# leggedrobotics/delora

Measured on AMD Instinct MI355X. Metric: training scan-pairs/sec, KITTI 64x2048 range images, higher is better.
Workload: dtype f32; 1 GPU; KITTI-shaped 64x2048, batch=8 pairs/GPU, raw scans of ~141k points (ragged, raster order), steps rotate over 8 distinct HBM-resident batches, online normals, ResNet pose CNN (11.9M params, identity-pretrained state), Adam; BASELINE configs[1]; global_batch=8, parallelism=dp1, cnn=fp32, cnn_impl=hip trunk: fp32 MFMA, fused Winograd F(2x2,3x3) + direct implicit GEMM, channels_last=False, hip_graph=False, distinct_batches=8, priming_steps=8

## Files before the change

delora_amd/_lib.py:

```python
import ctypes
import os

_HERE = os.path.dirname(os.path.abspath(__file__))
LIB_PATH = os.path.join(_HERE, "csrc", "libdelora_hip.so")
ABI_VERSION = 10


class DeloraHipError(RuntimeError):
    pass


class SensorStruct(ctypes.Structure):
    _fields_ = [("H", ctypes.c_int32), ("W", ctypes.c_int32),
                ("hfov0", ctypes.c_double), ("hfov1", ctypes.c_double),
                ("vfov0", ctypes.c_double), ("vfov1", ctypes.c_double)]


_vp, _i32, _i64, _u32, _f32, _sz = (ctypes.c_void_p, ctypes.c_int32, ctypes.c_int64, ctypes.c_uint32,
                                    ctypes.c_float, ctypes.c_size_t)
_SP = ctypes.POINTER(SensorStruct)

SIGNATURES = {
    "dl_abi_version": (_i32, []),
    "dl_last_error": (ctypes.c_char_p, []),
# ... 70 lines not shown
    "dl_channel_scale_bwd_act_nhwc_t": (_i32, [_vp, _vp, _vp, _i32, _i32, _i32, _i32, _i32, _vp, _vp]),
    "dl_tower_wide_drop_f32": (_i32, [_vp, _vp, ctypes.c_double, _i32, _i32, _i32, _i32, _i32, _vp, _vp]),
    "dl_tower_wide_drop_bwd_f32": (_i32, [_vp, _vp, _vp, ctypes.c_double, _i32, _i32, _i32, _i32, _i32, _i32, _vp, _vp]),
    "dl_mean_hw_nhwc_h": (_i32, [_vp, _i32, _i32, _i32, _i32, _vp, _vp]),
    "dl_mean_hw_bwd_act_h": (_i32, [_vp, _vp, _i32, _i32, _i32, _i32, _i32, _vp, _vp]),
    "dl_conv2d_wgrad_h_workspace_bytes": (_sz, [_i32, _i32, _i32, _i32, _i32, _i32, _i32, _i32]),
    "dl_conv2d_wgrad_nhwc_h": (_i32, [_vp, _vp, _vp, _vp, _i32, _i32, _i32, _i32, _i32, _i32, _i32, _i32, _i32, _vp]),
    "dl_wgrad_batch_plan": (_i64, [_vp, _vp, _i32, _i32, _i32, _vp]),
    "dl_wino_wgrad3x3_batch_workspace_bytes": (_sz, [_vp, _i32]),
    "dl_wino_wgrad3x3_batch_nhwc_f32": (_i32, [_vp, _i32, _vp, _vp]),
    "dl_conv2d_wgrad_batch_workspace_bytes": (_sz, [_vp, _i32]),
    "dl_conv2d_wgrad_batch_nhwc_f32": (_i32, [_vp, _i32, _vp, _vp]),
    "dl_conv2d_wgrad_batch_h_workspace_bytes": (_sz, [_vp, _i32]),
    "dl_conv2d_wgrad_batch_nhwc_h": (_i32, [_vp, _i32, _vp, _i32, _vp]),
    "dl_conv_plan_describe": (_i32, [_i32, _i32, _i32, _i32, _i32, _i32, _i32, _i32, _i32, _i32, _i32, _i32, ctypes.c_char_p, _sz]),
    "dl_profile_begin": (_i32, [_i32, ctypes.c_char_p]),
    "dl_profile_end": (_i32, [_vp, _i32, ctypes.POINTER(ctypes.c_int32), ctypes.POINTER(ctypes.c_int32)]),
    "dl_profile_pause": (_i32, [_i32]),
}


class WinoLayer(ctypes.Structure):
    _fields_ = [("w", ctypes.c_void_p), ("u_fwd", ctypes.c_void_p), ("u_bwd", ctypes.c_void_p), ("K", ctypes.c_int32), ("C", ctypes.c_int32)]


WINO_BATCH = 16


class HeadsParams(ctypes.Structure):
    _fields_ = [(n, ctypes.c_void_p) for n in ("fc_w", "fc_b", "r1_w", "r1_b", "r3_w", "r3_b", "t1_w", "t1_b", "t3_w", "t3_b")]
# ... 38 lines not shown
    rows = (ProfileRow * capacity)()
    n, untimed = ctypes.c_int32(), ctypes.c_int32()
    check(load().dl_profile_end(ctypes.cast(rows, ctypes.c_void_p), capacity, ctypes.byref(n), ctypes.byref(untimed)), "dl_profile_end")
    out = [{"name": rows[i].name.decode(), "launches": rows[i].launches, "ms": rows[i].ms, "flop": rows[i].flop, "bytes": rows[i].bytes}
           for i in range(min(n.value, capacity))]
    return out, untimed.value

PLAN_CONV, PLAN_DGRAD_STRIDED, PLAN_WINO_CONV, PLAN_WGRAD, PLAN_WGRAD_BATCH, PLAN_WINO_WGRAD, PLAN_WINO_WGRAD_BATCH = range(7)


def conv_plan(op, dtype, N, H, W, C, K, ksize=3, sh=1, sw=1, mode=0, cu_count=0):
    buf = ctypes.create_string_buffer(4096)
    check(load().dl_conv_plan_describe(int(op), int(dtype), int(N), int(H), int(W), int(C), int(K), int(ksize), int(sh), int(sw),
                                       int(mode), int(cu_count), buf, len(buf)), "dl_conv_plan_describe")
    return buf.value.decode().split("\n")


_lib = None


def load():
    global _lib
    if _lib is not None:
        return _lib
    if not os.path.exists(LIB_PATH):
        raise DeloraHipError(
            f"{LIB_PATH} is missing: build it with `python -c 'import __graft_entry__ as g; g.build()'` "
            f"or `make -C delora_amd/csrc`. The geometry path has no fallback implementation.")
    import torch
    try:
# ... 17 lines not shown
```

delora_amd/csrc/abi.hip:

```cpp
#include <stdarg.h>
#include <stdint.h>
#include <stdio.h>
#include <stdlib.h>
#include <string.h>
#include <cxxabi.h>

#include <atomic>
#include <map>
#include <mutex>
#include <string>
#include <vector>

#include "common.h"

thread_local char g_dl_err[256] = {0};

int dl_fail(int code, const char* fmt, ...) {
  va_list ap;
  va_start(ap, fmt);
  vsnprintf(g_dl_err, sizeof(g_dl_err), fmt, ap);
  va_end(ap);
  return code;
}

// ... 133 lines not shown
  free(full);
  char tail[96];
  const int m = snprintf(tail, sizeof(tail), " grid=%ux%ux%u block=%u", grid.x, grid.y, grid.z, block.x);
  dl_plan_append(tail, (size_t)m);
}

void dl_plan_note(const char* fmt, ...) {
  char text[96] = " ";
  va_list ap;
  va_start(ap, fmt);
  const int m = vsnprintf(text + 1, sizeof(text) - 1, fmt, ap);
  va_end(ap);
  if (m > 0) dl_plan_append(text, (size_t)(m < (int)sizeof(text) - 2 ? m + 1 : sizeof(text) - 1));
}

extern "C" int dl_abi_version(void) { return DL_ABI_VERSION; }
extern "C" const char* dl_last_error(void) { return g_dl_err; }

namespace {
struct ProfAgg { int launches = 0; double flop = 0, bytes = 0; std::vector<int> ev; };
struct Profiler {
  std::mutex mu;
  std::atomic<bool> open{false};
  std::atomic<bool> paused{false};
  std::vector<hipEvent_t> ev;
  int used = 0, skipped = 0;
  std::string only;
  std::map<std::string, ProfAgg> rows;
};
Profiler g_prof;
// ... 68 lines not shown
```

delora_amd/csrc/common.h:

```cpp
#pragma once
#include <hip/hip_runtime.h>
#include <stdint.h>

#include "../../include/delora_hip.h"

#define DL_WAVE 64
#define DL_BLOCK 256

struct SensorK {
  int H, W, HW;
  float hf0f, hspanf, wm1f;
  float vf0f, vspanf, hm1f;
  double hf0, hres, vf0, vres;
  float tol_u, tol_v;
};

static inline SensorK make_sensor(const dl_sensor* s) {
  SensorK k;
  k.H = s->H; k.W = s->W; k.HW = s->H * s->W;
  k.hf0f = (float)s->hfov0; k.hspanf = (float)(s->hfov1 - s->hfov0); k.wm1f = (float)(s->W - 1);
  k.vf0f = (float)s->vfov0; k.vspanf = (float)(s->vfov1 - s->vfov0); k.hm1f = (float)(s->H - 1);
  k.hf0 = s->hfov0; k.hres = (s->hfov1 - s->hfov0) / (double)(s->W - 1);
  k.vf0 = s->vfov0; k.vres = (s->vfov1 - s->vfov0) / (double)(s->H - 1);
  k.tol_u = (float)(3e-6 * fabs((double)k.wm1f / (double)k.hspanf) + 2.4e-7 * (double)s->W);
// ... 39 lines not shown
  p = __builtin_fmaf(p, t, 0.020650655031204224f);
  p = __builtin_fmaf(p, t, -0.05374353006482124f);
  p = __builtin_fmaf(p, t, 0.13331492245197296f);
  p = __builtin_fmaf(p, t, -0.3333328366279602f);
  const float lo = __builtin_fmaf(ax * t, p, ax);
  const float e = __builtin_amdgcn_exp2f(ax * 2.885390081777927f);
  const float hi = __builtin_fmaf(__builtin_amdgcn_rcpf(e + 1.f), -2.f, 1.f);
  return __builtin_copysignf(ax < 0.625f ? lo : hi, x);
}

extern thread_local char g_dl_err[256];
int dl_fail(int code, const char* fmt, ...);
int dl_check_launch(const char* what);
void dl_plan_batch(const int* tiles, const int* chunks, int n, int machines, int partial_cost, int* nslabs);
int dl_fill_words(void* p, uint32_t value, size_t n_words, hipStream_t st);

#include <hip/hip_ext.h>
struct DlProfTag {
  const char* kernel;
  const char* pass;
  int N, H, W, C, K;
  int ks, sh, sw;
  double flop;
  double bytes;
};
bool dl_prof_is_open();
void dl_prof_events(const DlProfTag& tag, hipEvent_t* e0, hipEvent_t* e1);

struct DlPlanSink {
  char* buf;
// ... 26 lines not shown
```

delora_amd/csrc/conv.hip:

```cpp
#include <type_traits>

#include "common.h"
#include "conv_geom.h"

typedef float f32x16 __attribute__((ext_vector_type(16)));
typedef float f32x4 __attribute__((ext_vector_type(4)));

__device__ __forceinline__ __amdgpu_buffer_rsrc_t cv_rsrc(const float* base, unsigned bytes) {
  return __builtin_amdgcn_make_buffer_rsrc(const_cast<float*>(base), 0, (int)bytes, 0x00020000);
}
__device__ __forceinline__ f32x4 cv_ld16(__amdgpu_buffer_rsrc_t rs, unsigned voff, unsigned soff) {
  return __builtin_bit_cast(f32x4, __builtin_amdgcn_raw_buffer_load_b128(rs, (int)voff, (int)soff, 0));
}
#define CV_ZERO_OFF 0x80000000u

#define CV_THREADS 256
#define CV_EPI_ADD 1u
#define CV_EPI_ACT 2u
#define CV_EPI_DACT 4u
#define CV_EPI_ADD_GRID 8u
#define CV_ACT_NONE 0
#define CV_ACT_TANH 1
#define CV_ACT_RELU 2

// ... 15 lines not shown
  if (act == CV_ACT_TANH) return dl_tanh(v);
  if (act == CV_ACT_RELU) return v < 0.f ? 0.f : v;
  return v;
}
__device__ __forceinline__ float cv_dact(float y, int act) {
  if (act == CV_ACT_TANH) return 1.f - y * y;
  if (act == CV_ACT_RELU) return y <= 0.f ? 0.f : 1.f;
  return 1.f;
}

__device__ __forceinline__ int cv_xcd_swizzle(int id, int n) {
  const int q = n / 8, r = n % 8, xcd = id % 8, k = id / 8;
  return (xcd < r ? xcd * (q + 1) : r * (q + 1) + (xcd - r) * q) + k;
}

template <int BM, int BN, int CK, int TW, class G, bool BT, int WGN>
#ifndef CV_MINWAVES
#define CV_MINWAVES 2
#endif
__global__ __launch_bounds__(CV_THREADS, CV_MINWAVES) void k_conv_f32(ConvArgs a) {
  constexpr int TH = BM / TW;
  constexpr int SH = G::ISH, SW = G::ISW;
  constexpr int RH = (TH - 1) * SH + G::EH, RW = (TW - 1) * SW + G::EW;
  constexpr int S = CK + 4;
  constexpr int TAPS = G::NT;
  constexpr int C4 = CK / 4;
  constexpr int IN_FLOATS = RH * RW * S;
  constexpr int W_FLOATS = BT ? TAPS * CK * BN : TAPS * BN * S;
  constexpr int NI = RH * RW * C4;
  constexpr int NW = BT ? CK * TAPS * (BN / 4) : BN * TAPS * C4;
  constexpr int NI_IT = (NI + CV_THREADS - 1) / CV_THREADS, NW_IT = (NW + CV_THREADS - 1) / CV_THREADS;
  constexpr int WGM = 4 / WGN;
  constexpr int WM = BM / 32 / WGM, WN = BN / 32 / WGN;
  static_assert(BM % TW == 0 && BM % (32 * WGM) == 0 && BN % (32 * WGN) == 0 && CK % 8 == 0, "tile shape");
  static_assert(TAPS > 0, "a stride phase without taps has no launch");
  static_assert((S / 4) % 2 == 1, "pixel stride must be 4*odd floats");
  constexpr int EPW = WN * 32, ES = EPW + 4;
  constexpr int LDS_HOLD = (BM == 256 && TW == 128 && CK == 8 && BT) ? 160 * 1024 / 3 / 4 + 16 : 0;
  constexpr int LDS_USED = IN_FLOATS + W_FLOATS > 4 * 32 * ES ? IN_FLOATS + W_FLOATS : 4 * 32 * ES;
  constexpr int LDS_FLOATS = LDS_USED > LDS_HOLD ? LDS_USED : LDS_HOLD;
  __shared__ __attribute__((aligned(16))) float lds[LDS_FLOATS];
  float* in_lds = lds;
  float* w_lds = lds + IN_FLOATS;

  const int tid = threadIdx.x, lane = tid & 63, wave = tid >> 6;
  const int li = lane & 31, half = lane >> 5;
  const int wm = wave / WGN, wn = wave % WGN;
  const int KT = a.K / BN;
  const int tiles_w = (a.Wo + TW - 1) / TW, tiles_h = (a.Ho + TH - 1) / TH;
  const int ntiles = a.N * tiles_h * tiles_w * KT;
  const int t = cv_xcd_swizzle(blockIdx.x, ntiles);
  const int kt = t % KT;
  int pt = t / KT;
  const int tw_i = pt % tiles_w; pt /= tiles_w;
  const int th_i = pt % tiles_h;
  const int n = pt / tiles_h;
  const int ho0 = th_i * TH, wo0 = tw_i * TW, k0 = kt * BN;
  const int h_base = ho0 * SH + G::H0, w_base = wo0 * SW + G::W0;
  const float* xn = a.x + (size_t)n * a.H * a.W * a.C;

  const unsigned x_bytes = (unsigned)(a.H * a.W * a.C) * 4u, w_bytes = (unsigned)(a.K * a.C * G::WTAPS) * 4u;
  const __amdgpu_buffer_rsrc_t x_rs = cv_rsrc(xn, x_bytes), w_rs = cv_rsrc(a.w, w_bytes);
  const unsigned x_zero = CV_ZERO_OFF;
  unsigned in_g[NI_IT];
  int in_l[NI_IT];
#pragma unroll
  for (int it = 0; it < NI_IT; ++it) {
    const int q = min(tid + it * CV_THREADS, NI - 1);
    const int c4 = q % C4, pc = q / C4;
    const int col = pc % RW, row = pc / RW;
    const int h = h_base + row;
    int w = w_base + col;
    const bool col_in = w >= 0 && w < a.W;
    w = w < 0 ? w + a.W : w;
    w = w >= a.W ? w - a.W : w;
    in_l[it] = pc * S + c4 * 4;
    in_g[it] = (h >= 0 && h < a.H && (a.wrap ? w < a.W : col_in)) ? (unsigned)((h * a.W + w) * a.C + c4 * 4) * 4u : x_zero;
  }
  unsigned w_g[NW_IT];
  int w_l[NW_IT];
#pragma unroll
  for (int it = 0; it < NW_IT; ++it) {
    const int q = min(tid + it * CV_THREADS, NW - 1);
    if (!BT) {
      const int c4 = q % C4, t2 = q / C4;
      const int tap = t2 % TAPS, kk = t2 / TAPS;
      w_g[it] = (unsigned)(((k0 + kk) * G::WTAPS + G::wt(tap)) * a.C + c4 * 4) * 4u;
      w_l[it] = (tap * BN + kk) * S + c4 * 4;
    } else {
      const int co4 = q % (BN / 4), t2 = q / (BN / 4);
      const int tap = t2 % TAPS, kr = t2 / TAPS;
      w_g[it] = (unsigned)((kr * G::WTAPS + G::wt(tap)) * a.K + k0 + co4 * 4) * 4u;
      w_l[it] = (tap * CK + kr) * BN + co4 * 4;
    }
  }

  f32x16 acc[WM][WN];
#pragma unroll
  for (int i = 0; i < WM; ++i)
#pragma unroll
    for (int j = 0; j < WN; ++j)
#pragma unroll
      for (int r = 0; r < 16; ++r) acc[i][j][r] = 0.f;

  int a_off[WM];
#pragma unroll
  for (int mi = 0; mi < WM; ++mi) {
    const int p = (wm * WM + mi) * 32 + li;
    const int th = p / TW, tw = p % TW;
    a_off[mi] = ((th * SH) * RW + tw * SW) * S + half * 4;
  }

  f32x4 in_r[NI_IT], w_r[NW_IT];
#define CV_FETCH(C0)                                                                                                      \
  {                                                                                                                       \
    const unsigned xs_ = (unsigned)(C0) * 4u, ws_ = BT ? (unsigned)((C0) * G::WTAPS * a.K) * 4u : xs_;          \
    _Pragma("unroll") for (int it = 0; it < NI_IT; ++it) in_r[it] = cv_ld16(x_rs, in_g[it], xs_);                         \
    _Pragma("unroll") for (int it = 0; it < NW_IT; ++it) w_r[it] = cv_ld16(w_rs, w_g[it], ws_);                           \
  }
#define CV_STAGE()                                                                                                        \
  {                                                                                                                       \
    _Pragma("unroll") for (int it = 0; it < NI_IT; ++it) *reinterpret_cast<f32x4*>(in_lds + in_l[it]) = in_r[it];         \
    _Pragma("unroll") for (int it = 0; it < NW_IT; ++it) *reinterpret_cast<f32x4*>(w_lds + w_l[it]) = w_r[it];            \
  }

  CV_FETCH(0)
  CV_STAGE()
  __syncthreads();
  for (int c0 = 0; c0 < a.C; c0 += CK) {
    const bool more = c0 + CK < a.C;
    if (more) CV_FETCH(c0 + CK)
#ifdef CV_OLD_LOOP
#pragma unroll
    for (int tap = 0; tap < TAPS; ++tap) {
#pragma unroll
      for (int kq = 0; kq < CK / 8; ++kq) {
        float4 af[WM];
#pragma unroll
        for (int mi = 0; mi < WM; ++mi)
          af[mi] = *reinterpret_cast<const float4*>(in_lds + a_off[mi] + (G::dh(tap) * RW + G::dw(tap)) * S + kq * 8);
        float bf[WN][4];
#pragma unroll
        for (int ni = 0; ni < WN; ++ni) {
          const int col = (wn * WN + ni) * 32 + li;
          if (!BT) {
            const float4 v = *reinterpret_cast<const float4*>(w_lds + (tap * BN + col) * S + kq * 8 + half * 4);
            bf[ni][0] = v.x; bf[ni][1] = v.y; bf[ni][2] = v.z; bf[ni][3] = v.w;
          } else {
#pragma unroll
            for (int j = 0; j < 4; ++j) bf[ni][j] = w_lds[(tap * CK + kq * 8 + half * 4 + j) * BN + col];
          }
        }
#pragma unroll
        for (int j = 0; j < 4; ++j)
#pragma unroll
          for (int mi = 0; mi < WM; ++mi) {
            const float av = j == 0 ? af[mi].x : (j == 1 ? af[mi].y : (j == 2 ? af[mi].z : af[mi].w));
#pragma unroll
            for (int ni = 0; ni < WN; ++ni)
              acc[mi][ni] = __builtin_amdgcn_mfma_f32_32x32x2f32(av, bf[ni][j], acc[mi][ni], 0, 0, 0);
          }
      }
    }
#else
    constexpr int KQ = CK / 8, NSTEP = TAPS * KQ;
    float4 af[2][WM];
    float bf[2][WN][4];
    auto load_frags = [&](int step, int buf) {
      const int tap = step / KQ, kq = step % KQ;
#pragma unroll
      for (int mi = 0; mi < WM; ++mi)
        af[buf][mi] = *reinterpret_cast<const float4*>(in_lds + a_off[mi] + (G::dh(tap) * RW + G::dw(tap)) * S + kq * 8);
#pragma unroll
      for (int ni = 0; ni < WN; ++ni) {
        const int col = (wn * WN + ni) * 32 + li;
        if (!BT) {
          const float4 v = *reinterpret_cast<const float4*>(w_lds + (tap * BN + col) * S + kq * 8 + half * 4);
          bf[buf][ni][0] = v.x; bf[buf][ni][1] = v.y; bf[buf][ni][2] = v.z; bf[buf][ni][3] = v.w;
        } else {
#pragma unroll
          for (int j = 0; j < 4; ++j) bf[buf][ni][j] = w_lds[(tap * CK + kq * 8 + half * 4 + j) * BN + col];
        }
      }
    };
    load_frags(0, 0);
#pragma unroll
    for (int step = 0; step < NSTEP; ++step) {
      const int cur = step & 1;
      if (step + 1 < NSTEP) load_frags(step + 1, cur ^ 1);
#pragma unroll
      for (int j = 0; j < 4; ++j)
#pragma unroll
        for (int mi = 0; mi < WM; ++mi) {
          const float av = j == 0 ? af[cur][mi].x : (j == 1 ? af[cur][mi].y : (j == 2 ? af[cur][mi].z : af[cur][mi].w));
#pragma unroll
          for (int ni = 0; ni < WN; ++ni)
            acc[mi][ni] = __builtin_amdgcn_mfma_f32_32x32x2f32(av, bf[cur][ni][j], acc[mi][ni], 0, 0, 0);
        }
#ifndef CV_NO_SGB
      if (step + 1 < NSTEP) __builtin_amdgcn_sched_group_barrier(0x100, WM + (BT ? 4 * WN : WN), 0);
      __builtin_amdgcn_sched_group_barrier(0x008, 4 * WM * WN, 0);
#endif
    }
#endif
    __syncthreads();
    if (more) {
      CV_STAGE()
      __syncthreads();
    }
  }

  __syncthreads();
  float* ep = lds + wave * (32 * ES);
  const unsigned out_n = (unsigned)(n * a.Hout * a.Wout), grid_n = (unsigned)(n * a.Ho * a.Wo);
  const unsigned k_lane = (unsigned)(k0 + wn * EPW);
  const bool f_add = a.epi & CV_EPI_ADD, f_act = a.epi & CV_EPI_ACT, f_dact = a.epi & CV_EPI_DACT;
  const bool f_addg = a.epi & CV_EPI_ADD_GRID;
#pragma unroll
  for (int mi = 0; mi < WM; ++mi) {
#pragma unroll
    for (int ni = 0; ni < WN; ++ni)
#pragma unroll
      for (int r = 0; r < 16; ++r) ep[((r & 3) + 8 * (r >> 2) + 4 * half) * ES + ni * 32 + li] = acc[mi][ni][r];
#pragma unroll 2
    for (int q = lane; q < 32 * (EPW / 4); q += 64) {
      const int row = q / (EPW / 4), c4 = q % (EPW / 4);
      const int p = (wm * WM + mi) * 32 + row;
      const int th = p / TW, tw = p % TW;
      const int oh = (ho0 + th) * G::OSH + G::OPH, ow = (wo0 + tw) * G::OSW + G::OPW;
      if (ho0 + th >= a.Ho || wo0 + tw >= a.Wo || oh >= a.Hout || ow >= a.Wout) continue;
      const unsigned o = (out_n + (unsigned)(oh * a.Wout + ow)) * (unsigned)a.K + k_lane + c4 * 4;
      float4 v = *reinterpret_cast<const float4*>(ep + row * ES + c4 * 4);
      if (a.seam && (ow == 0 || ow == a.Wout - 1)) {
        const float4 t = *reinterpret_cast<const float4*>(a.seam + ((unsigned)((n * a.Hout + oh) * 2 + (ow != 0)) * (unsigned)a.K + k_lane + c4 * 4));
        v.x += t.x; v.y += t.y; v.z += t.z; v.w += t.w;
      }
      if (f_addg) {
        const float4 t = *reinterpret_cast<const float4*>(a.add + ((grid_n + (unsigned)((ho0 + th) * a.Wo + (wo0 + tw))) * (unsigned)a.K + k_lane + c4 * 4));
        v.x += t.x; v.y += t.y; v.z += t.z; v.w += t.w;
      }
      if (f_add) {
        const float4 t = *reinterpret_cast<const float4*>(a.add + o);
        v.x += t.x; v.y += t.y; v.z += t.z; v.w += t.w;
      }
      if (f_act) { v.x = cv_act(v.x, a.act); v.y = cv_act(v.y, a.act); v.z = cv_act(v.z, a.act); v.w = cv_act(v.w, a.act); }
      if (f_dact) {
        const float4 t = *reinterpret_cast<const float4*>(a.dsrc + o);
        v.x *= cv_dact(t.x, a.act); v.y *= cv_dact(t.y, a.act); v.z *= cv_dact(t.z, a.act); v.w *= cv_dact(t.w, a.act);
      }
      *reinterpret_cast<float4*>(a.y + o) = v;
    }
  }
}

#undef CV_FETCH
#undef CV_STAGE

struct WgArgs {
  const float* x;
  const float* g;
  float* part;
  int N, H, W, C, K, Ho, Wo, chunks_per_slab, nslabs;
};
template <int BMK, int BNC, int PK, int SH, int SW, int KS, bool FAST>
__device__ __forceinline__ void wgrad_f32_body(const float* __restrict__ x, const float* __restrict__ g, float* __restrict__ part, int N, int H,
                                               int W, int C, int K, int Ho, int Wo, int chunks_per_slab, int nslabs, const int blk) {
  constexpr int PAD = (KS - 1) / 2;
  constexpr int TAPS = KS * KS;
  constexpr int RW = (PK - 1) * SW + KS;
  constexpr int X_FLOATS = KS * RW * BNC, G_FLOATS = PK * BMK;
  constexpr int NX = KS * RW * (BNC / 4), NG = PK * (BMK / 4);
// ... 223 lines not shown
  f32x4 s = {0.f, 0.f, 0.f, 0.f};
  int k = 0;
  for (; k + 8 <= nslabs; k += 8) {
    f32x4 v[8];
#pragma unroll
    for (int u = 0; u < 8; ++u) v[u] = __builtin_nontemporal_load(reinterpret_cast<const f32x4*>(part + (size_t)(k + u) * count + i));
#pragma unroll
    for (int u = 0; u < 8; ++u) s += v[u];
  }
  for (; k < nslabs; ++k) s += __builtin_nontemporal_load(reinterpret_cast<const f32x4*>(part + (size_t)k * count + i));
  *reinterpret_cast<f32x4*>(dw + i) = s;
}


template <int BM, int BN, int CK, int TW, class G, bool BT, int WGN>
static int launch_conv(const ConvArgs& a, hipStream_t st) {
  constexpr int TH = BM / TW;
  if (a.K % BN || a.C % CK) return 1;
  const int ntiles = a.N * ((a.Ho + TH - 1) / TH) * ((a.Wo + TW - 1) / TW) * (a.K / BN);
  const double px_ = (double)a.N * a.Ho * a.Wo;
  constexpr int ks_ = G::WTAPS == 9 ? 3 : 1;
  const DlProfTag tag{"k_conv_f32", BT ? "dgrad" : "fwd", a.N, a.H, a.W, a.C, a.K, ks_, BT ? G::OSH : G::ISH, BT ? G::OSW : G::ISW, 2.0 * px_ * a.K * a.C * G::NT,
                      4.0 * ((double)a.N * a.H * a.W * a.C + px_ * a.K + (double)G::WTAPS * a.K * a.C)};
  DL_LAUNCH(tag, (k_conv_f32<BM, BN, CK, TW, G, BT, WGN>), dim3(ntiles), dim3(CV_THREADS), st, a);
  return 0;
}

#ifndef CV_BN
#define CV_BN 64
#endif
#ifndef CV_CK
#define CV_CK 16
#endif
#ifndef CV_WGN
#define CV_WGN 2
#endif

#ifdef CV_TUNE
int g_cv_variant = 0;
// ... 397 lines not shown
```

delora_amd/csrc/conv_geom.h:

```cpp
#pragma once

template <int KS_, int SH_, int SW_>
struct GeomConv {
  static constexpr int NT = KS_ * KS_, WTAPS = KS_ * KS_, ISH = SH_, ISW = SW_;
  static constexpr int H0 = -((KS_ - 1) / 2), W0 = -((KS_ - 1) / 2), EH = KS_, EW = KS_;
  static constexpr int OSH = 1, OSW = 1, OPH = 0, OPW = 0;
  static constexpr int dh(int t) { return t / KS_; }
  static constexpr int dw(int t) { return t % KS_; }
  static constexpr int wt(int t) { return t; }
};

template <int KS_, int S_, int P_>
struct DgradAxis {
  static constexpr int PAD = (KS_ - 1) / 2;
  static constexpr bool valid(int r) { return (P_ + PAD - r) % S_ == 0; }
  static constexpr int off(int r) { return (P_ + PAD - r) / S_; }
  static constexpr int count() { int n = 0; for (int r = 0; r < KS_; ++r) n += valid(r) ? 1 : 0; return n; }
  static constexpr int tap(int i) { int n = 0; for (int r = 0; r < KS_; ++r) if (valid(r)) { if (n == i) return r; ++n; } return 0; }
  static constexpr int lo() { int m = 99; for (int r = 0; r < KS_; ++r) if (valid(r) && off(r) < m) m = off(r); return m; }
  static constexpr int hi() { int m = -99; for (int r = 0; r < KS_; ++r) if (valid(r) && off(r) > m) m = off(r); return m; }
};

template <int KS_, int SH_, int SW_, int PH_, int PW_, bool SO_>
struct GeomDgrad {
  using AH = DgradAxis<KS_, SH_, PH_>;
  using AW = DgradAxis<KS_, SW_, PW_>;
  static constexpr int NR = AH::count(), NS = AW::count();
  static constexpr int NT = NR * NS, WTAPS = KS_ * KS_, ISH = 1, ISW = 1;
  static constexpr int H0 = AH::lo(), W0 = AW::lo(), EH = AH::hi() - AH::lo() + 1, EW = AW::hi() - AW::lo() + 1;
  static constexpr int OSH = SO_ ? SH_ : 1, OSW = SO_ ? SW_ : 1, OPH = SO_ ? PH_ : 0, OPW = SO_ ? PW_ : 0;
  static constexpr int dh(int t) { return AH::off(AH::tap(t / NS)) - H0; }
  static constexpr int dw(int t) { return AW::off(AW::tap(t % NS)) - W0; }
  static constexpr int wt(int t) { return AH::tap(t / NS) * KS_ + AW::tap(t % NS); }
};
```

include/delora_hip.h:

```cpp
#ifndef DELORA_HIP_H
#define DELORA_HIP_H

#include <stddef.h>
#include <stdint.h>

#ifdef __cplusplus
extern "C" {
#endif

#define DL_ABI_VERSION 10

typedef void* dl_stream;

typedef enum {
  DL_OK = 0,
  DL_ERR_INVALID_ARGUMENT = -1,
  DL_ERR_LAUNCH = -2,
  DL_ERR_UNSUPPORTED = -3
} dl_status;

typedef struct {
  int32_t H;
  int32_t W;
  double hfov0, hfov1;
// ... 236 lines not shown
int dl_quat_to_T_bwd(const float* quaternion, const float* grad_T, int32_t B, float eps, float* grad_translation,
                     float* grad_quaternion, dl_stream stream);

int dl_mean_hw_nhwc_f32(const float* x, int32_t N, int32_t P, int32_t C, float* y, dl_stream stream);

#define DL_PLAN_CONV 0
#define DL_PLAN_DGRAD_STRIDED 1
#define DL_PLAN_WINO_CONV 2
#define DL_PLAN_WGRAD 3
#define DL_PLAN_WGRAD_BATCH 4
#define DL_PLAN_WINO_WGRAD 5
#define DL_PLAN_WINO_WGRAD_BATCH 6
int dl_conv_plan_describe(int32_t op, int32_t dtype, int32_t N, int32_t H, int32_t W, int32_t C, int32_t K, int32_t ksize,
                          int32_t stride_h, int32_t stride_w, int32_t mode, int32_t cu_count, char* buf, size_t buf_bytes);

typedef struct {
  char name[96];
  int32_t launches;
  double ms, flop, bytes;
} dl_profile_row;
int dl_profile_begin(int32_t max_launches, const char* only_kernel );
int dl_profile_pause(int32_t paused);
int dl_profile_end(dl_profile_row* rows, int32_t capacity, int32_t* count, int32_t* untimed);

#ifdef __cplusplus
}
#endif
#endif
```

Before: 666.5 scan-pairs/s.

## Make direct conv kernel persistent with cross-tile prefetch and compact strided staging

Turns the direct implicit-GEMM conv kernel into a persistent kernel. The grid is capped at CU count times resident blocks, and each workgroup loops over tiles, prefetching the next tile's first chunk while it finishes the current one. Input offsets are precomputed relative to the tile, with a fast path for interior tiles. Stride-only 1x1 geometry stages a compact LDS footprint, and the epilogue writes grouped vectors. This aims to cut launch tail effects, per-tile prologue cost and LDS waste, at the cost of more registers and more complex control flow, plus an optional runtime grid cap knob.

```diff
diff --git a/delora_amd/_lib.py b/delora_amd/_lib.py
--- a/delora_amd/_lib.py
+++ b/delora_amd/_lib.py
@@ -108,6 +108,7 @@
     "dl_conv2d_wgrad_batch_h_workspace_bytes": (_sz, [_vp, _i32]),
     "dl_conv2d_wgrad_batch_nhwc_h": (_i32, [_vp, _i32, _vp, _i32, _vp]),
     "dl_conv_plan_describe": (_i32, [_i32, _i32, _i32, _i32, _i32, _i32, _i32, _i32, _i32, _i32, _i32, _i32, ctypes.c_char_p, _sz]),
+    "dl_conv_direct_grid_cap": (_i32, [_i32]),
     "dl_profile_begin": (_i32, [_i32, ctypes.c_char_p]),
     "dl_profile_end": (_i32, [_vp, _i32, ctypes.POINTER(ctypes.c_int32), ctypes.POINTER(ctypes.c_int32)]),
     "dl_profile_pause": (_i32, [_i32]),
@@ -176,6 +177,10 @@
     check(load().dl_conv_plan_describe(int(op), int(dtype), int(N), int(H), int(W), int(C), int(K), int(ksize), int(sh), int(sw),
                                        int(mode), int(cu_count), buf, len(buf)), "dl_conv_plan_describe")
     return buf.value.decode().split("\n")
+
+
+def conv_direct_grid_cap(max_workgroups):
+    check(load().dl_conv_direct_grid_cap(int(max_workgroups)), "dl_conv_direct_grid_cap")
 
 
 _lib = None
diff --git a/delora_amd/csrc/abi.hip b/delora_amd/csrc/abi.hip
--- a/delora_amd/csrc/abi.hip
+++ b/delora_amd/csrc/abi.hip
@@ -171,6 +171,27 @@
   if (m > 0) dl_plan_append(text, (size_t)(m < (int)sizeof(text) - 2 ? m + 1 : sizeof(text) - 1));
 }
 
+int dl_cu_count() {
+  if (g_dl_plan && g_dl_plan->cu_count > 0) return g_dl_plan->cu_count;
+  static std::atomic<int> cache[64];
+  int dev = 0;
+  if (hipGetDevice(&dev) != hipSuccess || dev < 0 || dev >= 64) dev = 0;
+  int cus = cache[dev].load(std::memory_order_relaxed);
+  if (cus <= 0) {
+    if (hipDeviceGetAttribute(&cus, hipDeviceAttributeMultiprocessorCount, dev) != hipSuccess || cus <= 0) cus = 256;
+    cache[dev].store(cus, std::memory_order_relaxed);
+  }
+  return cus;
+}
+
+static std::atomic<int> g_conv_grid_cap{0};
+int dl_conv_grid_cap() { return g_conv_grid_cap.load(std::memory_order_relaxed); }
+extern "C" int dl_conv_direct_grid_cap(int32_t max_workgroups) {
+  if (max_workgroups < 0) return dl_fail(DL_ERR_INVALID_ARGUMENT, "dl_conv_direct_grid_cap: %d workgroups", max_workgroups);
+  g_conv_grid_cap.store(max_workgroups, std::memory_order_relaxed);
+  return DL_OK;
+}
+
 extern "C" int dl_abi_version(void) { return DL_ABI_VERSION; }
 extern "C" const char* dl_last_error(void) { return g_dl_err; }
 
diff --git a/delora_amd/csrc/common.h b/delora_amd/csrc/common.h
--- a/delora_amd/csrc/common.h
+++ b/delora_amd/csrc/common.h
@@ -77,6 +77,8 @@
 int dl_check_launch(const char* what);
 void dl_plan_batch(const int* tiles, const int* chunks, int n, int machines, int partial_cost, int* nslabs);
 int dl_fill_words(void* p, uint32_t value, size_t n_words, hipStream_t st);
+int dl_cu_count();
+int dl_conv_grid_cap();
 
 #include <hip/hip_ext.h>
 struct DlProfTag {
diff --git a/delora_amd/csrc/conv.hip b/delora_amd/csrc/conv.hip
--- a/delora_amd/csrc/conv.hip
+++ b/delora_amd/csrc/conv.hip
@@ -1,3 +1,5 @@
+#include <algorithm>
+#include <atomic>
 #include <type_traits>
 
 #include "common.h"
@@ -53,6 +55,17 @@
   return (xcd < r ? xcd * (q + 1) : r * (q + 1) + (xcd - r) * q) + k;
 }
 
+template <class G>
+constexpr bool cv_compact() { return G::EH == 1 && G::EW == 1 && (G::ISH > 1 || G::ISW > 1); }
+template <int BM, int BN, int CK, int TW, class G, bool BT>
+constexpr int cv_lds_floats() {
+  constexpr int TH = BM / TW, LSH = cv_compact<G>() ? 1 : G::ISH, LSW = cv_compact<G>() ? 1 : G::ISW;
+  constexpr int RH = (TH - 1) * LSH + G::EH, RW = (TW - 1) * LSW + G::EW, S = CK + 4;
+  constexpr int USED = RH * RW * S + (BT ? G::NT * CK * BN : G::NT * BN * S);
+  constexpr int HOLD = (BM == 256 && TW == 128 && CK == 8 && BT) ? 160 * 1024 / 3 / 4 + 16 : 0;
+  return USED > HOLD ? USED : HOLD;
+}
+
 template <int BM, int BN, int CK, int TW, class G, bool BT, int WGN>
 #ifndef CV_MINWAVES
 #define CV_MINWAVES 2
@@ -60,12 +73,14 @@
 __global__ __launch_bounds__(CV_THREADS, CV_MINWAVES) void k_conv_f32(ConvArgs a) {
   constexpr int TH = BM / TW;
   constexpr int SH = G::ISH, SW = G::ISW;
-  constexpr int RH = (TH - 1) * SH + G::EH, RW = (TW - 1) * SW + G::EW;
+  constexpr bool COMPACT = cv_compact<G>();
+  constexpr int LSH = COMPACT ? 1 : SH, LSW = COMPACT ? 1 : SW;
+  constexpr int GSH = COMPACT ? SH : 1, GSW = COMPACT ? SW : 1;
+  constexpr int RH = (TH - 1) * LSH + G::EH, RW = (TW - 1) * LSW + G::EW;
   constexpr int S = CK + 4;
   constexpr int TAPS = G::NT;
   constexpr int C4 = CK / 4;
   constexpr int IN_FLOATS = RH * RW * S;
-  constexpr int W_FLOATS = BT ? TAPS * CK * BN : TAPS * BN * S;
   constexpr int NI = RH * RW * C4;
   constexpr int NW = BT ? CK * TAPS * (BN / 4) : BN * TAPS * C4;
   constexpr int NI_IT = (NI + CV_THREADS - 1) / CV_THREADS, NW_IT = (NW + CV_THREADS - 1) / CV_THREADS;
@@ -74,11 +89,11 @@
   static_assert(BM % TW == 0 && BM % (32 * WGM) == 0 && BN % (32 * WGN) == 0 && CK % 8 == 0, "tile shape");
   static_assert(TAPS > 0, "a stride phase without taps has no launch");
   static_assert((S / 4) % 2 == 1, "pixel stride must be 4*odd floats");
-  constexpr int EPW = WN * 32, ES = EPW + 4;
-  constexpr int LDS_HOLD = (BM == 256 && TW == 128 && CK == 8 && BT) ? 160 * 1024 / 3 / 4 + 16 : 0;
-  constexpr int LDS_USED = IN_FLOATS + W_FLOATS > 4 * 32 * ES ? IN_FLOATS + W_FLOATS : 4 * 32 * ES;
-  constexpr int LDS_FLOATS = LDS_USED > LDS_HOLD ? LDS_USED : LDS_HOLD;
-  __shared__ __attribute__((aligned(16))) float lds[LDS_FLOATS];
+  static_assert(RH < 256 && RW < 4096 && C4 < 16, "packed item coordinates");
+  constexpr int EPW = WN * 32;
+  constexpr bool PREFETCH = !(BM == 256 && CK == 16);
+  constexpr int EG = 2;
+  __shared__ __attribute__((aligned(16))) float lds[cv_lds_floats<BM, BN, CK, TW, G, BT>()];
   float* in_lds = lds;
   float* w_lds = lds + IN_FLOATS;
 
@@ -88,33 +103,21 @@
   const int KT = a.K / BN;
   const int tiles_w = (a.Wo + TW - 1) / TW, tiles_h = (a.Ho + TH - 1) / TH;
   const int ntiles = a.N * tiles_h * tiles_w * KT;
-  const int t = cv_xcd_swizzle(blockIdx.x, ntiles);
-  const int kt = t % KT;
-  int pt = t / KT;
-  const int tw_i = pt % tiles_w; pt /= tiles_w;
-  const int th_i = pt % tiles_h;
-  const int n = pt / tiles_h;
-  const int ho0 = th_i * TH, wo0 = tw_i * TW, k0 = kt * BN;
-  const int h_base = ho0 * SH + G::H0, w_base = wo0 * SW + G::W0;
-  const float* xn = a.x + (size_t)n * a.H * a.W * a.C;
 
   const unsigned x_bytes = (unsigned)(a.H * a.W * a.C) * 4u, w_bytes = (unsigned)(a.K * a.C * G::WTAPS) * 4u;
-  const __amdgpu_buffer_rsrc_t x_rs = cv_rsrc(xn, x_bytes), w_rs = cv_rsrc(a.w, w_bytes);
+  const __amdgpu_buffer_rsrc_t w_rs = cv_rsrc(a.w, w_bytes);
+  __amdgpu_buffer_rsrc_t x_rs;
   const unsigned x_zero = CV_ZERO_OFF;
-  unsigned in_g[NI_IT];
-  int in_l[NI_IT];
+  unsigned in_g[NI_IT], in_rel[NI_IT];
+  int in_l[NI_IT], in_rc[NI_IT];
 #pragma unroll
   for (int it = 0; it < NI_IT; ++it) {
     const int q = min(tid + it * CV_THREADS, NI - 1);
     const int c4 = q % C4, pc = q / C4;
     const int col = pc % RW, row = pc / RW;
-    const int h = h_base + row;
-    int w = w_base + col;
-    const bool col_in = w >= 0 && w < a.W;
-    w = w < 0 ? w + a.W : w;
-    w = w >= a.W ? w - a.W : w;
     in_l[it] = pc * S + c4 * 4;
-    in_g[it] = (h >= 0 && h < a.H && (a.wrap ? w < a.W : col_in)) ? (unsigned)((h * a.W + w) * a.C + c4 * 4) * 4u : x_zero;
+    in_rc[it] = (row << 16) | (col << 4) | c4;
+    in_rel[it] = (unsigned)(((row * GSH) * a.W + col * GSW) * a.C + c4 * 4) * 4u;
   }
   unsigned w_g[NW_IT];
   int w_l[NW_IT];
@@ -124,36 +127,58 @@
     if (!BT) {
       const int c4 = q % C4, t2 = q / C4;
       const int tap = t2 % TAPS, kk = t2 / TAPS;
-      w_g[it] = (unsigned)(((k0 + kk) * G::WTAPS + G::wt(tap)) * a.C + c4 * 4) * 4u;
+      w_g[it] = (unsigned)((kk * G::WTAPS + G::wt(tap)) * a.C + c4 * 4) * 4u;
       w_l[it] = (tap * BN + kk) * S + c4 * 4;
     } else {
       const int co4 = q % (BN / 4), t2 = q / (BN / 4);
       const int tap = t2 % TAPS, kr = t2 / TAPS;
-      w_g[it] = (unsigned)((kr * G::WTAPS + G::wt(tap)) * a.K + k0 + co4 * 4) * 4u;
+      w_g[it] = (unsigned)((kr * G::WTAPS + G::wt(tap)) * a.K + co4 * 4) * 4u;
       w_l[it] = (tap * CK + kr) * BN + co4 * 4;
     }
   }
-
-  f32x16 acc[WM][WN];
-#pragma unroll
-  for (int i = 0; i < WM; ++i)
-#pragma unroll
-    for (int j = 0; j < WN; ++j)
-#pragma unroll
-      for (int r = 0; r < 16; ++r) acc[i][j][r] = 0.f;
 
   int a_off[WM];
 #pragma unroll
   for (int mi = 0; mi < WM; ++mi) {
     const int p = (wm * WM + mi) * 32 + li;
     const int th = p / TW, tw = p % TW;
-    a_off[mi] = ((th * SH) * RW + tw * SW) * S + half * 4;
-  }
-
+    a_off[mi] = ((th * LSH) * RW + tw * LSW) * S + half * 4;
+  }
+
+  int nx_n, nx_ho0, nx_wo0, nx_k0;
+  unsigned wk_off;
+#define CV_TILE(ID)                                                                                                       \
+  {                                                                                                                       \
+    const int t_ = cv_xcd_swizzle((ID), ntiles);                                                                          \
+    int pt_ = t_ / KT;                                                                                                    \
+    nx_k0 = (t_ % KT) * BN;                                                                                               \
+    nx_wo0 = (pt_ % tiles_w) * TW; pt_ /= tiles_w;                                                                        \
+    nx_ho0 = (pt_ % tiles_h) * TH;                                                                                        \
+    nx_n = pt_ / tiles_h;                                                                                                 \
+    const int hb_ = nx_ho0 * SH + G::H0, wb_ = nx_wo0 * SW + G::W0;                                                       \
+    x_rs = cv_rsrc(a.x + (size_t)nx_n * a.H * a.W * a.C, x_bytes);                                                        \
+    wk_off = BT ? (unsigned)nx_k0 * 4u : (unsigned)(nx_k0 * G::WTAPS * a.C) * 4u;                                         \
+    if (hb_ >= 0 && hb_ + (RH - 1) * GSH < a.H && wb_ >= 0 && wb_ + (RW - 1) * GSW < a.W) {                               \
+      const unsigned b_ = (unsigned)((hb_ * a.W + wb_) * a.C) * 4u;                                                       \
+      _Pragma("unroll") for (int it = 0; it < NI_IT; ++it) in_g[it] = in_rel[it] + b_;                                    \
+    } else {                                                                                                              \
+      _Pragma("unroll") for (int it = 0; it < NI_IT; ++it) {                                                              \
+        const int h = hb_ + (in_rc[it] >> 16) * GSH;                                                                      \
+        int w = wb_ + ((in_rc[it] >> 4) & 0xfff) * GSW;                                                                   \
+        const bool col_in = w >= 0 && w < a.W;                                                                            \
+        w = w < 0 ? w + a.W : w;                                                                                          \
+        w = w >= a.W ? w - a.W : w;                                                                                       \
+                       \
+        in_g[it] = (h >= 0 && h < a.H && (a.wrap ? w < a.W : col_in)) ? (unsigned)((h * a.W + w) * a.C + (in_rc[it] & 15) * 4) * 4u : x_zero; \
+      }                                                                                                                   \
+    }                                                                                                                     \
+  }
+
+  f32x16 acc[WM][WN];
   f32x4 in_r[NI_IT], w_r[NW_IT];
 #define CV_FETCH(C0)                                                                                                      \
   {                                                                                                                       \
-    const unsigned xs_ = (unsigned)(C0) * 4u, ws_ = BT ? (unsigned)((C0) * G::WTAPS * a.K) * 4u : xs_;          \
+    const unsigned xs_ = (unsigned)(C0) * 4u, ws_ = (BT ? (unsigned)((C0) * G::WTAPS * a.K) * 4u : xs_) + wk_off;    \
     _Pragma("unroll") for (int it = 0; it < NI_IT; ++it) in_r[it] = cv_ld16(x_rs, in_g[it], xs_);                         \
     _Pragma("unroll") for (int it = 0; it < NW_IT; ++it) w_r[it] = cv_ld16(w_rs, w_g[it], ws_);                           \
   }
@@ -162,138 +187,150 @@
     _Pragma("unroll") for (int it = 0; it < NI_IT; ++it) *reinterpret_cast<f32x4*>(in_lds + in_l[it]) = in_r[it];         \
     _Pragma("unroll") for (int it = 0; it < NW_IT; ++it) *reinterpret_cast<f32x4*>(w_lds + w_l[it]) = w_r[it];            \
   }
-
+  constexpr int KQ = CK / 8, NSTEP = TAPS * KQ;
+  const f32x16 zero16 = {0.f, 0.f, 0.f, 0.f, 0.f, 0.f, 0.f, 0.f, 0.f, 0.f, 0.f, 0.f, 0.f, 0.f, 0.f, 0.f};
+  float4 af[2][WM];
+  float bf[2][WN][4];
+  auto load_frags = [&](int step, int buf) {
+    const int tap = step / KQ, kq = step % KQ;
+#pragma unroll
+    for (int mi = 0; mi < WM; ++mi)
+      af[buf][mi] = *reinterpret_cast<const float4*>(in_lds + a_off[mi] + (G::dh(tap) * RW + G::dw(tap)) * S + kq * 8);
+#pragma unroll
+    for (int ni = 0; ni < WN; ++ni) {
+      const int col = (wn * WN + ni) * 32 + li;
+      if (!BT) {
+        const float4 v = *reinterpret_cast<const float4*>(w_lds + (tap * BN + col) * S + kq * 8 + half * 4);
+        bf[buf][ni][0] = v.x; bf[buf][ni][1] = v.y; bf[buf][ni][2] = v.z; bf[buf][ni][3] = v.w;
+      } else {
+#pragma unroll
+        for (int j = 0; j < 4; ++j) bf[buf][ni][j] = w_lds[(tap * CK + kq * 8 + half * 4 + j) * BN + col];
+      }
+    }
+  };
+#ifndef CV_NO_SGB
+#define CV_SGB(STEP)                                                                                                      \
+  if ((STEP) + 1 < NSTEP) __builtin_amdgcn_sched_group_barrier(0x100, WM + (BT ? 4 * WN : WN), 0);                        \
+  __builtin_amdgcn_sched_group_barrier(0x008, 4 * WM * WN, 0);
+#else
+#define CV_SGB(STEP)
+#endif
+#define CV_CHUNK(FIRST)                                                                                                   \
+  {                                                                                                                       \
+    load_frags(0, 0);                                                                                                     \
+    _Pragma("unroll") for (int step = 0; step < NSTEP; ++step) {                                                          \
+      const int cur = step & 1;                                                                                           \
+      if (step + 1 < NSTEP) load_frags(step + 1, cur ^ 1);                                                                \
+      _Pragma("unroll") for (int j = 0; j < 4; ++j)                                                                       \
+        _Pragma("unroll") for (int mi = 0; mi < WM; ++mi) {                                                               \
+          const float av = j == 0 ? af[cur][mi].x : (j == 1 ? af[cur][mi].y : (j == 2 ? af[cur][mi].z : af[cur][mi].w));  \
+          _Pragma("unroll") for (int ni = 0; ni < WN; ++ni)                                                               \
+            acc[mi][ni] = __builtin_amdgcn_mfma_f32_32x32x2f32(bf[cur][ni][j], av, (FIRST) && step == 0 && j == 0 ? zero16 : acc[mi][ni], 0, 0, 0); \
+        }                                                                                                                 \
+       \
+      CV_SGB(step)                                                                                                        \
+    }                                                                                                                     \
+  }
+
+  int id = blockIdx.x;
+  CV_TILE(id)
   CV_FETCH(0)
-  CV_STAGE()
-  __syncthreads();
-  for (int c0 = 0; c0 < a.C; c0 += CK) {
-    const bool more = c0 + CK < a.C;
-    if (more) CV_FETCH(c0 + CK)
-#ifdef CV_OLD_LOOP
-#pragma unroll
-    for (int tap = 0; tap < TAPS; ++tap) {
-#pragma unroll
-      for (int kq = 0; kq < CK / 8; ++kq) {
-        float4 af[WM];
-#pragma unroll
-        for (int mi = 0; mi < WM; ++mi)
-          af[mi] = *reinterpret_cast<const float4*>(in_lds + a_off[mi] + (G::dh(tap) * RW + G::dw(tap)) * S + kq * 8);
-        float bf[WN][4];
-#pragma unroll
-        for (int ni = 0; ni < WN; ++ni) {
-          const int col = (wn * WN + ni) * 32 + li;
-          if (!BT) {
-            const float4 v = *reinterpret_cast<const float4*>(w_lds + (tap * BN + col) * S + kq * 8 + half * 4);
-            bf[ni][0] = v.x; bf[ni][1] = v.y; bf[ni][2] = v.z; bf[ni][3] = v.w;
-          } else {
-#pragma unroll
-            for (int j = 0; j < 4; ++j) bf[ni][j] = w_lds[(tap * CK + kq * 8 + half * 4 + j) * BN + col];
+  const bool f_add = !G::STRIDED_DGRAD && (a.epi & CV_EPI_ADD), f_act = a.epi & CV_EPI_ACT, f_dact = a.epi & CV_EPI_DACT;
+  const bool f_addg = G::STRIDED_DGRAD && (a.epi & CV_EPI_ADD_GRID);
+  for (;;) {
+    const int n = nx_n, ho0 = nx_ho0, wo0 = nx_wo0, k0 = nx_k0;
+    CV_STAGE()
+    __syncthreads();
+    {
+      const bool more = CK < a.C;
+      if (more) CV_FETCH(CK)
+      CV_CHUNK(true)
+      __syncthreads();
+      if (more) {
+        CV_STAGE()
+        __syncthreads();
+      }
+    }
+    for (int c0 = CK; c0 < a.C; c0 += CK) {
+      const bool more = c0 + CK < a.C;
+      if (more) CV_FETCH(c0 + CK)
+      CV_CHUNK(false)
+      __syncthreads();
+      if (more) {
+        CV_STAGE()
+        __syncthreads();
+      }
+    }
+    id += gridDim.x;
+    const bool has_next = id < ntiles;
+    if (PREFETCH && has_next) {
+      CV_TILE(id)
+      CV_FETCH(0)
+    }
+
+    const unsigned out_n = (unsigned)(n * a.Hout * a.Wout), grid_n = (unsigned)(n * a.Ho * a.Wo);
+    const unsigned k_lane = (unsigned)(k0 + wn * EPW + half * 4);
+#pragma unroll
+    for (int mi = 0; mi < WM; ++mi) {
+      const int p = (wm * WM + mi) * 32 + li;
+      const int gh = ho0 + p / TW, gw = wo0 + p % TW;
+      const int oh = gh * G::OSH + G::OPH, ow = gw * G::OSW + G::OPW;
+      if (gh >= a.Ho || gw >= a.Wo || oh >= a.Hout || ow >= a.Wout) continue;
+      const unsigned o = (out_n + (unsigned)(oh * a.Wout + ow)) * (unsigned)a.K + k_lane;
+      const unsigned go = (grid_n + (unsigned)(gh * a.Wo + gw)) * (unsigned)a.K + k_lane;
+      const bool f_seam = G::OSW > 1 && a.seam && (ow == 0 || ow == a.Wout - 1);
+      const unsigned so = (unsigned)((n * a.Hout + oh) * 2 + (ow != 0)) * (unsigned)a.K + k_lane;
+#pragma unroll
+      for (int ni = 0; ni < WN; ++ni)
+#pragma unroll
+        for (int g0 = 0; g0 < 4; g0 += EG) {
+          const unsigned e = (unsigned)(ni * 32 + g0 * 8);
+          f32x4 v[EG], ts[EG], tg[EG], ta[EG], td[EG];
+          if (f_seam) {
+#pragma unroll
+            for (int g = 0; g < EG; ++g) ts[g] = *reinterpret_cast<const f32x4*>(a.seam + so + e + g * 8);
           }
+          if (f_addg) {
+#pragma unroll
+            for (int g = 0; g < EG; ++g) tg[g] = *reinterpret_cast<const f32x4*>(a.add + go + e + g * 8);
+          }
+          if (f_add) {
+#pragma unroll
+            for (int g = 0; g < EG; ++g) ta[g] = *reinterpret_cast<const f32x4*>(a.add + o + e + g * 8);
+          }
+          if (f_dact) {
+#pragma unroll
+            for (int g = 0; g < EG; ++g) td[g] = *reinterpret_cast<const f32x4*>(a.dsrc + o + e + g * 8);
+          }
+#pragma unroll
+          for (int g = 0; g < EG; ++g) {
+            const int r = 4 * (g0 + g);
+            v[g] = (f32x4){acc[mi][ni][r], acc[mi][ni][r + 1], acc[mi][ni][r + 2], acc[mi][ni][r + 3]};
+            if (f_seam) v[g] += ts[g];
+            if (f_addg) v[g] += tg[g];
+            if (f_add) v[g] += ta[g];
+            if (f_act) { v[g].x = cv_act(v[g].x, a.act); v[g].y = cv_act(v[g].y, a.act); v[g].z = cv_act(v[g].z, a.act); v[g].w = cv_act(v[g].w, a.act); }
+            if (f_dact) {
+              v[g].x *= cv_dact(td[g].x, a.act); v[g].y *= cv_dact(td[g].y, a.act); v[g].z *= cv_dact(td[g].z, a.act); v[g].w *= cv_dact(td[g].w, a.act);
+            }
+          }
+#pragma unroll
+          for (int g = 0; g < EG; ++g) *reinterpret_cast<f32x4*>(a.y + o + e + g * 8) = v[g];
         }
-#pragma unroll
-        for (int j = 0; j < 4; ++j)
-#pragma unroll
-          for (int mi = 0; mi < WM; ++mi) {
-            const float av = j == 0 ? af[mi].x : (j == 1 ? af[mi].y : (j == 2 ? af[mi].z : af[mi].w));
-#pragma unroll
-            for (int ni = 0; ni < WN; ++ni)
-              acc[mi][ni] = __builtin_amdgcn_mfma_f32_32x32x2f32(av, bf[ni][j], acc[mi][ni], 0, 0, 0);
-          }
-      }
-    }
-#else
-    constexpr int KQ = CK / 8, NSTEP = TAPS * KQ;
-    float4 af[2][WM];
-    float bf[2][WN][4];
-    auto load_frags = [&](int step, int buf) {
-      const int tap = step / KQ, kq = step % KQ;
-#pragma unroll
-      for (int mi = 0; mi < WM; ++mi)
-        af[buf][mi] = *reinterpret_cast<const float4*>(in_lds + a_off[mi] + (G::dh(tap) * RW + G::dw(tap)) * S + kq * 8);
-#pragma unroll
-      for (int ni = 0; ni < WN; ++ni) {
-        const int col = (wn * WN + ni) * 32 + li;
-        if (!BT) {
-          const float4 v = *reinterpret_cast<const float4*>(w_lds + (tap * BN + col) * S + kq * 8 + half * 4);
-          bf[buf][ni][0] = v.x; bf[buf][ni][1] = v.y; bf[buf][ni][2] = v.z; bf[buf][ni][3] = v.w;
-        } else {
-#pragma unroll
-          for (int j = 0; j < 4; ++j) bf[buf][ni][j] = w_lds[(tap * CK + kq * 8 + half * 4 + j) * BN + col];
-        }
-      }
-    };
-    load_frags(0, 0);
-#pragma unroll
-    for (int step = 0; step < NSTEP; ++step) {
-      const int cur = step & 1;
-      if (step + 1 < NSTEP) load_frags(step + 1, cur ^ 1);
-#pragma unroll
-      for (int j = 0; j < 4; ++j)
-#pragma unroll
-        for (int mi = 0; mi < WM; ++mi) {
-          const float av = j == 0 ? af[cur][mi].x : (j == 1 ? af[cur][mi].y : (j == 2 ? af[cur][mi].z : af[cur][mi].w));
-#pragma unroll
-          for (int ni = 0; ni < WN; ++ni)
-            acc[mi][ni] = __builtin_amdgcn_mfma_f32_32x32x2f32(av, bf[cur][ni][j], acc[mi][ni], 0, 0, 0);
-        }
-#ifndef CV_NO_SGB
-      if (step + 1 < NSTEP) __builtin_amdgcn_sched_group_barrier(0x100, WM + (BT ? 4 * WN : WN), 0);
-      __builtin_amdgcn_sched_group_barrier(0x008, 4 * WM * WN, 0);
-#endif
-    }
-#endif
-    __syncthreads();
-    if (more) {
-      CV_STAGE()
-      __syncthreads();
-    }
-  }
-
-  __syncthreads();
-  float* ep = lds + wave * (32 * ES);
-  const unsigned out_n = (unsigned)(n * a.Hout * a.Wout), grid_n = (unsigned)(n * a.Ho * a.Wo);
-  const unsigned k_lane = (unsigned)(k0 + wn * EPW);
-  const bool f_add = a.epi & CV_EPI_ADD, f_act = a.epi & CV_EPI_ACT, f_dact = a.epi & CV_EPI_DACT;
-  const bool f_addg = a.epi & CV_EPI_ADD_GRID;
-#pragma unroll
-  for (int mi = 0; mi < WM; ++mi) {
-#pragma unroll
-    for (int ni = 0; ni < WN; ++ni)
-#pragma unroll
-      for (int r = 0; r < 16; ++r) ep[((r & 3) + 8 * (r >> 2) + 4 * half) * ES + ni * 32 + li] = acc[mi][ni][r];
-#pragma unroll 2
-    for (int q = lane; q < 32 * (EPW / 4); q += 64) {
-      const int row = q / (EPW / 4), c4 = q % (EPW / 4);
-      const int p = (wm * WM + mi) * 32 + row;
-      const int th = p / TW, tw = p % TW;
-      const int oh = (ho0 + th) * G::OSH + G::OPH, ow = (wo0 + tw) * G::OSW + G::OPW;
-      if (ho0 + th >= a.Ho || wo0 + tw >= a.Wo || oh >= a.Hout || ow >= a.Wout) continue;
-      const unsigned o = (out_n + (unsigned)(oh * a.Wout + ow)) * (unsigned)a.K + k_lane + c4 * 4;
-      float4 v = *reinterpret_cast<const float4*>(ep + row * ES + c4 * 4);
-      if (a.seam && (ow == 0 || ow == a.Wout - 1)) {
-        const float4 t = *reinterpret_cast<const float4*>(a.seam + ((unsigned)((n * a.Hout + oh) * 2 + (ow != 0)) * (unsigned)a.K + k_lane + c4 * 4));
-        v.x += t.x; v.y += t.y; v.z += t.z; v.w += t.w;
-      }
-      if (f_addg) {
-        const float4 t = *reinterpret_cast<const float4*>(a.add + ((grid_n + (unsigned)((ho0 + th) * a.Wo + (wo0 + tw))) * (unsigned)a.K + k_lane + c4 * 4));
-        v.x += t.x; v.y += t.y; v.z += t.z; v.w += t.w;
-      }
-      if (f_add) {
-        const float4 t = *reinterpret_cast<const float4*>(a.add + o);
-        v.x += t.x; v.y += t.y; v.z += t.z; v.w += t.w;
-      }
-      if (f_act) { v.x = cv_act(v.x, a.act); v.y = cv_act(v.y, a.act); v.z = cv_act(v.z, a.act); v.w = cv_act(v.w, a.act); }
-      if (f_dact) {
-        const float4 t = *reinterpret_cast<const float4*>(a.dsrc + o);
-        v.x *= cv_dact(t.x, a.act); v.y *= cv_dact(t.y, a.act); v.z *= cv_dact(t.z, a.act); v.w *= cv_dact(t.w, a.act);
-      }
-      *reinterpret_cast<float4*>(a.y + o) = v;
-    }
-  }
-}
-
+    }
+    if (!has_next) break;
+    if (!PREFETCH) {
+      CV_TILE(id)
+      CV_FETCH(0)
+    }
+  }
+}
+
+#undef CV_TILE
 #undef CV_FETCH
 #undef CV_STAGE
+#undef CV_CHUNK
+#undef CV_SGB
 
 struct WgArgs {
   const float* x;
@@ -547,15 +584,38 @@
 
 
 template <int BM, int BN, int CK, int TW, class G, bool BT, int WGN>
+static int cv_resident() {
+  constexpr int lds_bytes = cv_lds_floats<BM, BN, CK, TW, G, BT>() * 4;
+  constexpr int by_lds = 160 * 1024 / lds_bytes;
+  constexpr int derived = by_lds > 8 ? 8 : (by_lds < CV_MINWAVES ? CV_MINWAVES : by_lds);
+  if (g_dl_plan && g_dl_plan->cu_count > 0) return derived;
+  static std::atomic<int> cache[64];
+  int dev = 0;
+  if (hipGetDevice(&dev) != hipSuccess || dev < 0 || dev >= 64) dev = 0;
+  int r = cache[dev].load(std::memory_order_relaxed);
+  if (r <= 0) {
+    if (hipOccupancyMaxActiveBlocksPerMultiprocessor(&r, k_conv_f32<BM, BN, CK, TW, G, BT, WGN>, CV_THREADS, 0) != hipSuccess || r <= 0) {
+      (void)hipGetLastError();
+      r = derived;
+    }
+    cache[dev].store(r, std::memory_order_relaxed);
+  }
+  return r;
+}
+
+template <int BM, int BN, int CK, int TW, class G, bool BT, int WGN>
 static int launch_conv(const ConvArgs& a, hipStream_t st) {
   constexpr int TH = BM / TW;
   if (a.K % BN || a.C % CK) return 1;
   const int ntiles = a.N * ((a.Ho + TH - 1) / TH) * ((a.Wo + TW - 1) / TW) * (a.K / BN);
+  int grid = std::min(ntiles, dl_cu_count() * cv_resident<BM, BN, CK, TW, G, BT, WGN>());
+  const int cap = dl_conv_grid_cap();
+  if (cap > 0 && grid > cap) grid = cap;
   const double px_ = (double)a.N * a.Ho * a.Wo;
   constexpr int ks_ = G::WTAPS == 9 ? 3 : 1;
   const DlProfTag tag{"k_conv_f32", BT ? "dgrad" : "fwd", a.N, a.H, a.W, a.C, a.K, ks_, BT ? G::OSH : G::ISH, BT ? G::OSW : G::ISW, 2.0 * px_ * a.K * a.C * G::NT,
                       4.0 * ((double)a.N * a.H * a.W * a.C + px_ * a.K + (double)G::WTAPS * a.K * a.C)};
-  DL_LAUNCH(tag, (k_conv_f32<BM, BN, CK, TW, G, BT, WGN>), dim3(ntiles), dim3(CV_THREADS), st, a);
+  DL_LAUNCH(tag, (k_conv_f32<BM, BN, CK, TW, G, BT, WGN>), dim3(grid), dim3(CV_THREADS), st, a);
   return 0;
 }
 
diff --git a/delora_amd/csrc/conv_geom.h b/delora_amd/csrc/conv_geom.h
--- a/delora_amd/csrc/conv_geom.h
+++ b/delora_amd/csrc/conv_geom.h
@@ -5,6 +5,7 @@
   static constexpr int NT = KS_ * KS_, WTAPS = KS_ * KS_, ISH = SH_, ISW = SW_;
   static constexpr int H0 = -((KS_ - 1) / 2), W0 = -((KS_ - 1) / 2), EH = KS_, EW = KS_;
   static constexpr int OSH = 1, OSW = 1, OPH = 0, OPW = 0;
+  static constexpr bool STRIDED_DGRAD = false;
   static constexpr int dh(int t) { return t / KS_; }
   static constexpr int dw(int t) { return t % KS_; }
   static constexpr int wt(int t) { return t; }
@@ -29,6 +30,7 @@
   static constexpr int NT = NR * NS, WTAPS = KS_ * KS_, ISH = 1, ISW = 1;
   static constexpr int H0 = AH::lo(), W0 = AW::lo(), EH = AH::hi() - AH::lo() + 1, EW = AW::hi() - AW::lo() + 1;
   static constexpr int OSH = SO_ ? SH_ : 1, OSW = SO_ ? SW_ : 1, OPH = SO_ ? PH_ : 0, OPW = SO_ ? PW_ : 0;
+  static constexpr bool STRIDED_DGRAD = SH_ > 1 || SW_ > 1;
   static constexpr int dh(int t) { return AH::off(AH::tap(t / NS)) - H0; }
   static constexpr int dw(int t) { return AW::off(AW::tap(t % NS)) - W0; }
   static constexpr int wt(int t) { return AH::tap(t / NS) * KS_ + AW::tap(t % NS); }
diff --git a/include/delora_hip.h b/include/delora_hip.h
--- a/include/delora_hip.h
+++ b/include/delora_hip.h
@@ -274,6 +274,8 @@
 int dl_conv_plan_describe(int32_t op, int32_t dtype, int32_t N, int32_t H, int32_t W, int32_t C, int32_t K, int32_t ksize,
                           int32_t stride_h, int32_t stride_w, int32_t mode, int32_t cu_count, char* buf, size_t buf_bytes);
 
+int dl_conv_direct_grid_cap(int32_t max_workgroups);
+
 typedef struct {
   char name[96];
   int32_t launches;
```

After: 669.3 scan-pairs/s (median of 6 runs). About the same (+0.4%).
